# pySTEPS/pysteps

Hardware: NVIDIA H100
Metric: Mpix/s advected (2048^2 frame, 12 leadtimes) (higher is better)
Workload: dtype f64 (trajectories, motion field, IDW); f32 precip in/out; u8/i16/f32 OpenCV-exact LK stages

## Files before the change

### pysteps_b200/csrc/lk_features.cu

```cuda
#include <math_constants.h>

#include "common.cuh"

namespace {

constexpr int TX = 32, TY = 8;

__global__ void __launch_bounds__(256)
masked_max_partial(const float *__restrict__ eig, const uint8_t *__restrict__ valid, size_t N,
                   float *__restrict__ part) {
    __shared__ float sm[8];
    float v = -CUDART_INF_F;
    const size_t stride = (size_t)gridDim.x * blockDim.x;
    for (size_t i = (size_t)blockIdx.x * blockDim.x + threadIdx.x; i < N; i += stride)
        if (!valid || valid[i]) v = fmaxf(v, eig[i]);
#pragma unroll
    for (int o = 16; o > 0; o >>= 1) v = fmaxf(v, __shfl_xor_sync(0xffffffffu, v, o));
    if ((threadIdx.x & 31) == 0) sm[threadIdx.x >> 5] = v;
    __syncthreads();
    if (threadIdx.x < 32) {
        v = threadIdx.x < 8 ? sm[threadIdx.x] : -CUDART_INF_F;
#pragma unroll
        for (int o = 4; o > 0; o >>= 1) v = fmaxf(v, __shfl_xor_sync(0xffffffffu, v, o));
        if (threadIdx.x == 0) part[blockIdx.x] = v;
    }
}

__global__ void __launch_bounds__(256)
masked_max_final(const float *__restrict__ part, int nparts, double quality, unsigned *__restrict__ state) {
    __shared__ float sm[8];
    float v = -CUDART_INF_F;
    for (int i = threadIdx.x; i < nparts; i += blockDim.x) v = fmaxf(v, part[i]);
#pragma unroll
    for (int o = 16; o > 0; o >>= 1) v = fmaxf(v, __shfl_xor_sync(0xffffffffu, v, o));
    if ((threadIdx.x & 31) == 0) sm[threadIdx.x >> 5] = v;
    __syncthreads();
    if (threadIdx.x == 0) {
        for (int i = 1; i < 8; i++) v = fmaxf(v, sm[i]);
        const double mx = (v == -CUDART_INF_F) ? 0.0 : (double)v;
        const float thr = (float)(mx * quality);
        state[0] = __float_as_uint(thr);
        state[1] = 0u;
        state[2] = (v == -CUDART_INF_F) ? 1u : 0u;
    }
}

__device__ __forceinline__ unsigned order_key(float v) {
    const unsigned u = __float_as_uint(v);
    return (u & 0x80000000u) ? ~u : (u | 0x80000000u);
}

__global__ void __launch_bounds__(TX *TY)
candidates_kernel(const float *__restrict__ eig, const uint8_t *__restrict__ valid, int h, int w,
                  unsigned *__restrict__ state, unsigned long long *__restrict__ keys, unsigned cap) {
    const int x = blockIdx.x * TX + threadIdx.x, y = blockIdx.y * TY + threadIdx.y;
    if (x < 1 || y < 1 || x >= w - 1 || y >= h - 1) return;
    const float thr = __uint_as_float(state[0]);
    const size_t i = (size_t)y * w + x;
    const float v = eig[i];
    if (!(v > thr) || v == 0.f) return;
    if (valid && !valid[i]) return;
    bool ismax = true;
#pragma unroll
    for (int dy = -1; dy <= 1; dy++)
#pragma unroll
        for (int dx = -1; dx <= 1; dx++) {
            float u = eig[(size_t)(y + dy) * w + (x + dx)];
            u = (u > thr) ? u : 0.f;
            ismax &= !(u > v);
        }
    if (!ismax) return;
    const unsigned slot = atomicAdd(&state[1], 1u);
    if (slot < cap) keys[slot] = ((unsigned long long)order_key(v) << 32) | (unsigned)i;
}

constexpr int SORT_BLOCK = 1024;
constexpr int SORT_TILE = 2 * SORT_BLOCK;

__device__ __forceinline__ void cmpswap_desc(unsigned long long &a, unsigned long long &b, bool desc) {
    if ((a < b) == desc) {
        const unsigned long long t = a; a = b; b = t;
    }
}

__global__ void __launch_bounds__(SORT_BLOCK)
bitonic_local_kernel(unsigned long long *__restrict__ keys, unsigned n, unsigned k_start, unsigned k_end) {
    __shared__ unsigned long long sm[SORT_TILE];
    const unsigned base = blockIdx.x * SORT_TILE;
    for (unsigned t = threadIdx.x; t < SORT_TILE; t += SORT_BLOCK) sm[t] = (base + t < n) ? keys[base + t] : 0ull;
    __syncthreads();
    for (unsigned k = k_start; k <= k_end; k <<= 1) {
        const unsigned jmax = (k_start == k_end && k_start > SORT_TILE) ? SORT_TILE / 2 : k / 2;
        for (unsigned j = (jmax < k / 2 ? jmax : k / 2); j > 0; j >>= 1) {
            const unsigned t = threadIdx.x;
            const unsigned lo = 2 * t - (t & (j - 1));
            const unsigned hi = lo + j;
            const bool desc = (((base + lo) & k) == 0);
            cmpswap_desc(sm[lo], sm[hi], desc);
            __syncthreads();
        }
    }
    for (unsigned t = threadIdx.x; t < SORT_TILE; t += SORT_BLOCK)
        if (base + t < n) keys[base + t] = sm[t];
}

__global__ void __launch_bounds__(256)
bitonic_global_kernel(unsigned long long *__restrict__ keys, unsigned n, unsigned k, unsigned j) {
    const unsigned t = blockIdx.x * blockDim.x + threadIdx.x;
    if (t >= n / 2) return;
    const unsigned lo = 2 * t - (t & (j - 1));
    const unsigned hi = lo + j;
    const bool desc = ((lo & k) == 0);
    unsigned long long a = keys[lo], b = keys[hi];
    if ((a < b) == desc) { keys[lo] = b; keys[hi] = a; }
}

constexpr int CELL_CAP = 8;

__device__ __forceinline__ bool too_close(float dx, float dy, double md2) {
    return (double)__fadd_rn(__fmul_rn(dx, dx), __fmul_rn(dy, dy)) < md2;
}

struct SelectParams {
    const unsigned long long *keys;
    const unsigned *state;
    unsigned cap;
    int h, w, max_corners;
    double md2;
    bool use_dist;
    int cell, gw, gh;
    int *cell_cnt;
    short2 *cell_pts;
    float *out_xy;
    int *out_count;
};

__global__ void __launch_bounds__(32) select_kernel(const SelectParams p) {
    const int lane = threadIdx.x;
    const unsigned ncand = min(p.state[1], p.cap);
    int accepted = 0;
    const bool limited = p.max_corners > 0;
    for (unsigned basei = 0; basei < ncand; basei += 32) {
        const unsigned ci = basei + lane;
        bool ok = ci < ncand;
        int x = 0, y = 0;
        if (ok) {
            const unsigned addr = (unsigned)(p.keys[ci] & 0xffffffffull);
            y = addr / p.w;
            x = addr - y * p.w;
        }
        const int xc = x / p.cell, yc = y / p.cell;
        if (ok && p.use_dist) {
            const int x1 = max(0, xc - 1), y1 = max(0, yc - 1);
            const int x2 = min(p.gw - 1, xc + 1), y2 = min(p.gh - 1, yc + 1);
            for (int yy = y1; yy <= y2 && ok; yy++)
                for (int xx = x1; xx <= x2 && ok; xx++) {
                    const int c = yy * p.gw + xx;
                    const int cnt = min(p.cell_cnt[c], CELL_CAP);
                    for (int q = 0; q < cnt; q++) {
                        const short2 pt = p.cell_pts[c * CELL_CAP + q];
                        if (too_close((float)(x - pt.x), (float)(y - pt.y), p.md2)) { ok = false; break; }
                    }
                }
        }
        for (int i = 0; i < 32; i++) {
            const bool oki = __shfl_sync(0xffffffffu, ok, i);
            const int xi = __shfl_sync(0xffffffffu, x, i), yi = __shfl_sync(0xffffffffu, y, i);
            if (oki && lane > i && ok && p.use_dist && too_close((float)(x - xi), (float)(y - yi), p.md2))
                ok = false;
        }
        const unsigned bal = __ballot_sync(0xffffffffu, ok);
        const int rank = __popc(bal & ((1u << lane) - 1u));
        const bool take = ok && (!limited || accepted + rank < p.max_corners);
        const int c = yc * p.gw + xc;
        int before = 0;
        for (int i = 0; i < 32; i++) {
            const int ci2 = __shfl_sync(0xffffffffu, c, i);
            const bool ti = __shfl_sync(0xffffffffu, take, i);
            if (ti && i < lane && ci2 == c) before++;
        }
        if (take) {
            const int o = accepted + rank;
            p.out_xy[2 * o] = (float)x;
            p.out_xy[2 * o + 1] = (float)y;
            if (p.use_dist) {
                const int slot = p.cell_cnt[c] + before;
                if (slot < CELL_CAP) p.cell_pts[c * CELL_CAP + slot] = make_short2((short)x, (short)y);
            }
        }
        __syncwarp();
        if (take && p.use_dist) atomicAdd(&p.cell_cnt[c], 1);
        __threadfence_block();
        __syncwarp();
        accepted += __popc(bal);
        if (limited && accepted >= p.max_corners) { accepted = p.max_corners; break; }
    }
    if (lane == 0) *p.out_count = accepted;
}

constexpr int SEL_WARPS = 8;
constexpr unsigned SEL_DONE = 0xffffffffu;

__global__ void __launch_bounds__(32 * SEL_WARPS) select_smem_kernel(const SelectParams p) {
    extern __shared__ unsigned cells[];
    const int lane = threadIdx.x & 31, warp = threadIdx.x >> 5;
    const int ncell = p.gw * p.gh;
    volatile unsigned *ctl = cells + ncell;
    for (int i = threadIdx.x; i < ncell + 2; i += 32 * SEL_WARPS) cells[i] = 0u;
    __syncthreads();
    const unsigned ncand = min(p.state[1], p.cap);
    const unsigned nbatch = (ncand + 31u) / 32u;
    const unsigned md2i = (unsigned)ceil(p.md2);
    const bool limited = p.max_corners > 0;
    for (unsigned b = warp; b < nbatch; b += SEL_WARPS) {
        const unsigned ci = b * 32u + lane;
        bool ok = ci < ncand;
        int x = 0, y = 0;
        if (ok) {
            const unsigned addr = (unsigned)(p.keys[ci] & 0xffffffffull);
            y = addr / p.w;
            x = addr - y * p.w;
        }
        const int xc = x / p.cell, yc = y / p.cell;
        unsigned close = 0u;
#pragma unroll 8
        for (int i = 0; i < 32; i++) {
            const int xi = __shfl_sync(0xffffffffu, x, i), yi = __shfl_sync(0xffffffffu, y, i);
            const int dx = x - xi, dy = y - yi;
            if (i < lane && (unsigned)(dx * dx) + (unsigned)(dy * dy) < md2i) close |= 1u << i;
        }
        int nidx[9];
#pragma unroll
        for (int k = 0; k < 9; k++) {
            const int xx = xc + k % 3 - 1, yy = yc + k / 3 - 1;
            nidx[k] = (ok && xx >= 0 && yy >= 0 && xx < p.gw && yy < p.gh) ? yy * p.gw + xx : -1;
        }
        unsigned tok;
        while ((tok = ctl[0]) != b && tok != SEL_DONE) {}
        if (tok == SEL_DONE) break;
        __syncwarp();
        int accepted = (int)ctl[1];
        unsigned wds[9], any = 0u;
#pragma unroll
        for (int k = 0; k < 9; k++) {
            wds[k] = nidx[k] >= 0 ? cells[nidx[k]] : 0u;
            any |= wds[k];
        }
        if (any) {
#pragma unroll
            for (int k = 0; k < 9; k++) {
                const unsigned wd = wds[k];
                const int cnt = wd & 3u;
                const int ox = (xc + k % 3 - 1) * p.cell, oy = (yc + k / 3 - 1) * p.cell;
                for (int q = 0; q < cnt; q++) {
                    const unsigned f = (wd >> (2 + 10 * q)) & 0x3ffu;
                    if (too_close((float)(x - (ox + (int)(f & 31u))), (float)(y - (oy + (int)(f >> 5))), p.md2))
                        ok = false;
                }
            }
        }
        const unsigned okmask = __ballot_sync(0xffffffffu, ok);
        close &= okmask;
        unsigned acc = __ballot_sync(0xffffffffu, ok && close == 0u);
        unsigned pend = okmask & ~acc;
        while (pend) {
            const int i = __ffs(pend) - 1;
            pend &= pend - 1;
            const bool oki = (__shfl_sync(0xffffffffu, close, i) & acc) == 0u;
            if (oki) acc |= 1u << i;
        }
        ok = (acc >> lane) & 1u;
        const unsigned bal = __ballot_sync(0xffffffffu, ok);
        const int rank = __popc(bal & ((1u << lane) - 1u));
        const bool take = ok && (!limited || accepted + rank < p.max_corners);
        if (take) {
            const int o = accepted + rank;
            p.out_xy[2 * o] = (float)x;
            p.out_xy[2 * o + 1] = (float)y;
        }
        const unsigned tmask = __ballot_sync(0xffffffffu, take);
        const int c = yc * p.gw + xc;
        if (take) {
            const unsigned grp = __match_any_sync(tmask, c);
            if (lane == __ffs(grp) - 1) {
                unsigned wd = cells[c];
                unsigned g = grp;
                while (g) {
                    const int j = __ffs(g) - 1;
                    g &= g - 1;
                    const int xj = __shfl_sync(grp, x, j), yj = __shfl_sync(grp, y, j);
                    const unsigned cnt = wd & 3u;
                    if (cnt < 3u) {
                        const unsigned f = (unsigned)(xj - xc * p.cell) | ((unsigned)(yj - yc * p.cell) << 5);
                        wd = (wd & ~3u) | (f << (2 + 10 * cnt)) | (cnt + 1u);
                    }
                }
                cells[c] = wd;
            } else {
                unsigned g = grp;
                while (g) {
                    const int j = __ffs(g) - 1;
                    g &= g - 1;
                    __shfl_sync(grp, x, j);
                    __shfl_sync(grp, y, j);
                }
            }
        }
        __syncwarp();
        accepted += __popc(bal);
        const bool full = limited && accepted >= p.max_corners;
        if (full) accepted = p.max_corners;
        __threadfence_block();
        if (lane == 0) {
            ctl[1] = (unsigned)accepted;
            __threadfence_block();
            ctl[0] = full ? SEL_DONE : b + 1u;
        }
        if (full) break;
    }
    __syncthreads();
    if (threadIdx.x == 0) *p.out_count = (int)ctl[1];
}

}

extern "C" int b200_good_features(const float *eig, const uint8_t *valid, int m, int n, int max_corners,
                                  double quality_level, double min_distance, float *out_xy,
                                  int *out_count, void *stream) {
    B200_REQUIRE(eig && out_xy && out_count && m >= 1 && n >= 1 && max_corners > 0, "bad arguments");
    B200_REQUIRE((int64_t)m * n < ((int64_t)1 << 31), "image too large");
    cudaStream_t s = (cudaStream_t)stream;
    const size_t N = (size_t)m * n;
    const int nparts = b200::num_sms() * 4;
    b200::Scratch part, state, keys, cellc, cellp;
    B200_CUDA(part.alloc(sizeof(float) * nparts, s));
    B200_CUDA(state.alloc(sizeof(unsigned) * 4, s));
    masked_max_partial<<<nparts, 256, 0, s>>>(eig, valid, N, (float *)part.p);
    B200_LAUNCH_CHECK();
    masked_max_final<<<1, 256, 0, s>>>((const float *)part.p, nparts, quality_level, (unsigned *)state.p);
    B200_LAUNCH_CHECK();
    const unsigned cap = (unsigned)N;
    size_t cap_pow2 = SORT_TILE;
    while (cap_pow2 < (size_t)cap) cap_pow2 <<= 1;
    B200_CUDA(keys.alloc(sizeof(unsigned long long) * cap_pow2, s));
    candidates_kernel<<<dim3(b200::ceil_div(n, TX), b200::ceil_div(m, TY)), dim3(TX, TY), 0, s>>>(
        eig, valid, m, n, (unsigned *)state.p, (unsigned long long *)keys.p, cap);
    B200_LAUNCH_CHECK();
    unsigned hstate[4];
    B200_CUDA(cudaMemcpyAsync(hstate, state.p, sizeof(hstate), cudaMemcpyDeviceToHost, s));
    B200_CUDA(cudaStreamSynchronize(s));
    unsigned ncand = hstate[1] < cap ? hstate[1] : cap;
    if (hstate[2]) ncand = 0;
    if (ncand == 0) {
        B200_CUDA(cudaMemsetAsync(out_count, 0, sizeof(int), s));
        return 0;
    }
    unsigned npow = SORT_TILE;
    while (npow < ncand) npow <<= 1;
    if (npow > ncand)
        B200_CUDA(cudaMemsetAsync((unsigned long long *)keys.p + ncand, 0,
                                  sizeof(unsigned long long) * (npow - ncand), s));
    unsigned long long *K = (unsigned long long *)keys.p;
    bitonic_local_kernel<<<npow / SORT_TILE, SORT_BLOCK, 0, s>>>(K, npow, 2, SORT_TILE);
    B200_LAUNCH_CHECK();
    for (unsigned k = 2 * SORT_TILE; k <= npow; k <<= 1) {
        for (unsigned j = k / 2; j >= SORT_TILE; j >>= 1) {
            bitonic_global_kernel<<<b200::ceil_div((int)(npow / 2), 256), 256, 0, s>>>(K, npow, k, j);
            B200_LAUNCH_CHECK();
        }
        bitonic_local_kernel<<<npow / SORT_TILE, SORT_BLOCK, 0, s>>>(K, npow, k, k);
        B200_LAUNCH_CHECK();
    }
    SelectParams sp;
    sp.keys = K;
    sp.state = (const unsigned *)state.p;
    sp.cap = ncand;
    sp.h = m; sp.w = n;
    sp.max_corners = max_corners;
    sp.md2 = min_distance * min_distance;
    sp.use_dist = min_distance >= 1.0;
    sp.cell = sp.use_dist ? (int)lrint(min_distance) : 1;
    sp.gw = (n + sp.cell - 1) / sp.cell;
    sp.gh = (m + sp.cell - 1) / sp.cell;
    const size_t ncell = (size_t)sp.gw * sp.gh;
    sp.out_xy = out_xy;
    sp.out_count = out_count;
    if (sp.use_dist && sp.cell <= 32 && ncell * sizeof(unsigned) <= 200 * 1024) {
        const size_t smem = (ncell + 2) * sizeof(unsigned);
        B200_CUDA(cudaFuncSetAttribute(select_smem_kernel, cudaFuncAttributeMaxDynamicSharedMemorySize, (int)smem));
        select_smem_kernel<<<1, 32 * SEL_WARPS, smem, s>>>(sp);
        B200_LAUNCH_CHECK();
        return 0;
    }
    B200_CUDA(cellc.alloc(sizeof(int) * ncell, s));
    B200_CUDA(cellp.alloc(sizeof(short2) * ncell * CELL_CAP, s));
    B200_CUDA(cudaMemsetAsync(cellc.p, 0, sizeof(int) * ncell, s));
    sp.cell_cnt = (int *)cellc.p;
    sp.cell_pts = (short2 *)cellp.p;
    sp.out_xy = out_xy;
    sp.out_count = out_count;
    select_kernel<<<1, 32, 0, s>>>(sp);
    B200_LAUNCH_CHECK();
    return 0;
}
```

Before: 19940.

## Replace full bitonic sort of corner candidates with radix top-k chunked selection

The full bitonic sort of every corner candidate is replaced by a radix-histogram top-k pass. It partitions the candidates into those above and those on a 12-bit threshold digit, then sorts only 2048-key chunks in shared memory inside a single fused select kernel. This also removes the device-to-host copy and stream synchronization that used to read the candidate count. The aim is to cut the many global bitonic kernel launches and the host stall in good-features-to-track. In exchange, selection now runs in one block, and every chunk after the first rescans all candidates, which costs more if many chunks are needed.

Result: faster. 20440, median of 6 (+2.5%).

```diff
diff --git a/pysteps_b200/csrc/lk_features.cu b/pysteps_b200/csrc/lk_features.cu
--- a/pysteps_b200/csrc/lk_features.cu
+++ b/pysteps_b200/csrc/lk_features.cu
@@ -5,6 +5,8 @@
 namespace {
 
 constexpr int TX = 32, TY = 8;
+constexpr int RADIX_BITS = 12;
+constexpr unsigned RADIX = 1u << RADIX_BITS;
 
 __global__ void __launch_bounds__(256)
 masked_max_partial(const float *__restrict__ eig, const uint8_t *__restrict__ valid, size_t N,
@@ -31,6 +33,7 @@
     __shared__ float sm[8];
     float v = -CUDART_INF_F;
     for (int i = threadIdx.x; i < nparts; i += blockDim.x) v = fmaxf(v, part[i]);
+    for (int i = 4 + threadIdx.x; i < 8 + (int)RADIX; i += blockDim.x) state[i] = 0u;
 #pragma unroll
     for (int o = 16; o > 0; o >>= 1) v = fmaxf(v, __shfl_xor_sync(0xffffffffu, v, o));
     if ((threadIdx.x & 31) == 0) sm[threadIdx.x >> 5] = v;
@@ -74,45 +77,188 @@
     if (slot < cap) keys[slot] = ((unsigned long long)order_key(v) << 32) | (unsigned)i;
 }
 
-constexpr int SORT_BLOCK = 1024;
-constexpr int SORT_TILE = 2 * SORT_BLOCK;
-
-__device__ __forceinline__ void cmpswap_desc(unsigned long long &a, unsigned long long &b, bool desc) {
-    if ((a < b) == desc) {
-        const unsigned long long t = a; a = b; b = t;
-    }
-}
-
-__global__ void __launch_bounds__(SORT_BLOCK)
-bitonic_local_kernel(unsigned long long *__restrict__ keys, unsigned n, unsigned k_start, unsigned k_end) {
-    __shared__ unsigned long long sm[SORT_TILE];
-    const unsigned base = blockIdx.x * SORT_TILE;
-    for (unsigned t = threadIdx.x; t < SORT_TILE; t += SORT_BLOCK) sm[t] = (base + t < n) ? keys[base + t] : 0ull;
-    __syncthreads();
-    for (unsigned k = k_start; k <= k_end; k <<= 1) {
-        const unsigned jmax = (k_start == k_end && k_start > SORT_TILE) ? SORT_TILE / 2 : k / 2;
-        for (unsigned j = (jmax < k / 2 ? jmax : k / 2); j > 0; j >>= 1) {
-            const unsigned t = threadIdx.x;
-            const unsigned lo = 2 * t - (t & (j - 1));
-            const unsigned hi = lo + j;
-            const bool desc = (((base + lo) & k) == 0);
-            cmpswap_desc(sm[lo], sm[hi], desc);
+constexpr int TOPK_THREADS = 1024;
+constexpr unsigned CHUNK = 2048;
+constexpr int PER_THREAD = RADIX / TOPK_THREADS;
+static_assert(RADIX * sizeof(unsigned) <= CHUNK * sizeof(unsigned long long), "the histogram aliases the chunk");
+static_assert(TOPK_THREADS == 32 * 32, "block_inclusive_scan: one warp scans the warp totals");
+
+constexpr int LOAD_BATCH = 8;
+
+__device__ __forceinline__ void load_keys(const unsigned long long *__restrict__ keys, unsigned ncand, unsigned b,
+                                          unsigned long long (&k)[LOAD_BATCH]) {
+#pragma unroll
+    for (int j = 0; j < LOAD_BATCH; j++) {
+        const unsigned i = b + j * TOPK_THREADS + threadIdx.x;
+        k[j] = i < ncand ? keys[i] : 0ull;
+    }
+}
+
+struct TopkShared {
+    unsigned wsum[32];
+    unsigned digit, above, bucket;
+    unsigned n;
+};
+
+__device__ __forceinline__ unsigned block_inclusive_scan(unsigned v, TopkShared &sh) {
+    const int lane = threadIdx.x & 31, warp = threadIdx.x >> 5;
+#pragma unroll
+    for (int o = 1; o < 32; o <<= 1) {
+        const unsigned t = __shfl_up_sync(0xffffffffu, v, o);
+        if (lane >= o) v += t;
+    }
+    if (lane == 31) sh.wsum[warp] = v;
+    __syncthreads();
+    if (warp == 0) {
+        unsigned w = sh.wsum[lane];
+#pragma unroll
+        for (int o = 1; o < 32; o <<= 1) {
+            const unsigned t = __shfl_up_sync(0xffffffffu, w, o);
+            if (lane >= o) w += t;
+        }
+        sh.wsum[lane] = w;
+    }
+    __syncthreads();
+    return v + (warp ? sh.wsum[warp - 1] : 0u);
+}
+
+__device__ void find_digit(const unsigned *hist, unsigned need, TopkShared &sh) {
+    unsigned c[PER_THREAD], s = 0u;
+#pragma unroll
+    for (int j = 0; j < PER_THREAD; j++) {
+        c[j] = hist[RADIX - 1 - PER_THREAD * threadIdx.x - j];
+        s += c[j];
+    }
+    const unsigned incl = block_inclusive_scan(s, sh);
+    unsigned above = incl - s;
+    if (above < need && incl >= need) {
+#pragma unroll
+        for (int j = 0; j < PER_THREAD; j++) {
+            if (above + c[j] >= need) {
+                sh.digit = RADIX - 1 - PER_THREAD * threadIdx.x - j;
+                sh.above = above;
+                sh.bucket = c[j];
+                break;
+            }
+            above += c[j];
+        }
+    }
+    __syncthreads();
+}
+
+__device__ unsigned long long chunk_bound(const unsigned long long *__restrict__ keys, unsigned nkeys,
+                                          unsigned long long hi, unsigned need, unsigned have, int used,
+                                          unsigned long long prefix, unsigned *hist, TopkShared &sh) {
+    unsigned long long pmask = used ? ~0ull << (64 - used) : 0ull;
+    while (have != need && used < 64) {
+        const int width = min(RADIX_BITS, 64 - used), shift = 64 - used - width;
+        const unsigned dmask = (1u << width) - 1u;
+        for (unsigned i = threadIdx.x; i < RADIX; i += TOPK_THREADS) hist[i] = 0u;
+        __syncthreads();
+        for (unsigned b = 0; b < nkeys; b += LOAD_BATCH * TOPK_THREADS) {
+            unsigned long long k[LOAD_BATCH];
+            load_keys(keys, nkeys, b, k);
+#pragma unroll
+            for (int j = 0; j < LOAD_BATCH; j++)
+                if (k[j] != 0ull && k[j] < hi && (k[j] & pmask) == prefix)
+                    atomicAdd(&hist[(unsigned)(k[j] >> shift) & dmask], 1u);
+        }
+        __syncthreads();
+        find_digit(hist, need, sh);
+        need -= sh.above;
+        have = sh.bucket;
+        prefix |= (unsigned long long)sh.digit << shift;
+        pmask |= (unsigned long long)dmask << shift;
+        used += width;
+        __syncthreads();
+    }
+    return prefix;
+}
+
+__device__ void append_keys(const unsigned long long *__restrict__ keys, unsigned nkeys, unsigned long long lo,
+                            unsigned long long hi, unsigned long long *chunk, TopkShared &sh) {
+    const int lane = threadIdx.x & 31;
+    for (unsigned b = 0; b < nkeys; b += LOAD_BATCH * TOPK_THREADS) {
+        unsigned long long k[LOAD_BATCH];
+        load_keys(keys, nkeys, b, k);
+#pragma unroll
+        for (int j = 0; j < LOAD_BATCH; j++) {
+            const unsigned bal = __ballot_sync(0xffffffffu, k[j] != 0ull && k[j] >= lo && k[j] < hi);
+            unsigned base = 0u;
+            if (lane == 0 && bal) base = atomicAdd(&sh.n, __popc(bal));
+            base = __shfl_sync(0xffffffffu, base, 0);
+            if ((bal >> lane) & 1u) chunk[base + __popc(bal & ((1u << lane) - 1u))] = k[j];
+        }
+    }
+    __syncthreads();
+}
+
+__device__ void sort_chunk(unsigned long long *chunk, unsigned n) {
+    unsigned npow = 2u;
+    while (npow < n) npow <<= 1;
+    for (unsigned i = n + threadIdx.x; i < npow; i += TOPK_THREADS) chunk[i] = 0ull;
+    __syncthreads();
+    for (unsigned k = 2; k <= npow; k <<= 1)
+        for (unsigned j = k >> 1; j > 0; j >>= 1) {
+            for (unsigned t = threadIdx.x; t < npow / 2; t += TOPK_THREADS) {
+                const unsigned a = 2 * t - (t & (j - 1));
+                const bool desc = (a & k) == 0;
+                const unsigned long long x = chunk[a], y = chunk[a + j];
+                if ((x < y) == desc) {
+                    chunk[a] = y;
+                    chunk[a + j] = x;
+                }
+            }
             __syncthreads();
         }
-    }
-    for (unsigned t = threadIdx.x; t < SORT_TILE; t += SORT_BLOCK)
-        if (base + t < n) keys[base + t] = sm[t];
-}
-
-__global__ void __launch_bounds__(256)
-bitonic_global_kernel(unsigned long long *__restrict__ keys, unsigned n, unsigned k, unsigned j) {
-    const unsigned t = blockIdx.x * blockDim.x + threadIdx.x;
-    if (t >= n / 2) return;
-    const unsigned lo = 2 * t - (t & (j - 1));
-    const unsigned hi = lo + j;
-    const bool desc = ((lo & k) == 0);
-    unsigned long long a = keys[lo], b = keys[hi];
-    if ((a < b) == desc) { keys[lo] = b; keys[hi] = a; }
+}
+
+constexpr int TOP_SHIFT = 64 - RADIX_BITS;
+
+__device__ __forceinline__ unsigned candidate_count(const unsigned *state, unsigned cap) {
+    return state[2] ? 0u : min(state[1], cap);
+}
+
+__global__ void __launch_bounds__(TOPK_THREADS)
+key_hist_kernel(const unsigned long long *__restrict__ keys, unsigned *__restrict__ state, unsigned cap) {
+    __shared__ unsigned h[RADIX];
+    const unsigned ncand = candidate_count(state, cap);
+    if (ncand <= CHUNK) return;
+    for (unsigned i = threadIdx.x; i < RADIX; i += TOPK_THREADS) h[i] = 0u;
+    __syncthreads();
+    for (unsigned i = blockIdx.x * TOPK_THREADS + threadIdx.x; i < ncand; i += gridDim.x * TOPK_THREADS)
+        atomicAdd(&h[(unsigned)(keys[i] >> TOP_SHIFT)], 1u);
+    __syncthreads();
+    for (unsigned i = threadIdx.x; i < RADIX; i += TOPK_THREADS)
+        if (h[i]) atomicAdd(&state[8 + i], h[i]);
+}
+
+__global__ void __launch_bounds__(TOPK_THREADS)
+key_partition_kernel(const unsigned long long *__restrict__ keys, unsigned *__restrict__ state, unsigned cap,
+                     unsigned long long *__restrict__ top, unsigned long long *__restrict__ edge) {
+    __shared__ unsigned h[RADIX];
+    __shared__ TopkShared sh;
+    const unsigned ncand = candidate_count(state, cap);
+    if (ncand <= CHUNK) return;
+    for (unsigned i = threadIdx.x; i < RADIX; i += TOPK_THREADS) h[i] = state[8 + i];
+    __syncthreads();
+    find_digit(h, CHUNK, sh);
+    const unsigned d0 = sh.digit;
+    if (blockIdx.x == 0 && threadIdx.x == 0) state[6] = d0;
+    const int lane = threadIdx.x & 31;
+    for (unsigned b = blockIdx.x * TOPK_THREADS; b < ncand; b += gridDim.x * TOPK_THREADS) {
+        const unsigned i = b + threadIdx.x;
+        const unsigned long long k = i < ncand ? keys[i] : 0ull;
+        const unsigned d = (unsigned)(k >> TOP_SHIFT);
+#pragma unroll
+        for (int side = 0; side < 2; side++) {
+            const unsigned bal = __ballot_sync(0xffffffffu, i < ncand && (side ? d == d0 : d > d0));
+            unsigned base = 0u;
+            if (lane == 0 && bal) base = atomicAdd(&state[4 + side], __popc(bal));
+            base = __shfl_sync(0xffffffffu, base, 0);
+            if ((bal >> lane) & 1u) (side ? edge : top)[base + __popc(bal & ((1u << lane) - 1u))] = k;
+        }
+    }
 }
 
 constexpr int CELL_CAP = 8;
@@ -125,6 +271,7 @@
     const unsigned long long *keys;
     const unsigned *state;
     unsigned cap;
+    const unsigned long long *top, *edge;
     int h, w, max_corners;
     double md2;
     bool use_dist;
@@ -135,17 +282,20 @@
     int *out_count;
 };
 
-__global__ void __launch_bounds__(32) select_kernel(const SelectParams p) {
-    const int lane = threadIdx.x;
-    const unsigned ncand = min(p.state[1], p.cap);
-    int accepted = 0;
+constexpr unsigned SEL_DONE = 0xffffffffu;
+
+__device__ void select_chunk_global(const SelectParams &p, const unsigned long long *keys, unsigned ncand,
+                                    volatile unsigned *ctl) {
+    const int lane = threadIdx.x & 31;
+    int accepted = (int)ctl[1];
     const bool limited = p.max_corners > 0;
+    bool full = false;
     for (unsigned basei = 0; basei < ncand; basei += 32) {
         const unsigned ci = basei + lane;
         bool ok = ci < ncand;
         int x = 0, y = 0;
         if (ok) {
-            const unsigned addr = (unsigned)(p.keys[ci] & 0xffffffffull);
+            const unsigned addr = (unsigned)(keys[ci] & 0xffffffffull);
             y = addr / p.w;
             x = addr - y * p.w;
         }
@@ -193,22 +343,19 @@
         __threadfence_block();
         __syncwarp();
         accepted += __popc(bal);
-        if (limited && accepted >= p.max_corners) { accepted = p.max_corners; break; }
-    }
-    if (lane == 0) *p.out_count = accepted;
+        if (limited && accepted >= p.max_corners) { accepted = p.max_corners; full = true; break; }
+    }
+    if (lane == 0) {
+        ctl[1] = (unsigned)accepted;
+        if (full) ctl[0] = SEL_DONE;
+    }
 }
 
 constexpr int SEL_WARPS = 8;
-constexpr unsigned SEL_DONE = 0xffffffffu;
-
-__global__ void __launch_bounds__(32 * SEL_WARPS) select_smem_kernel(const SelectParams p) {
-    extern __shared__ unsigned cells[];
+
+__device__ void select_chunk_smem(const SelectParams &p, const unsigned long long *keys, unsigned ncand,
+                                  unsigned *cells, volatile unsigned *ctl) {
     const int lane = threadIdx.x & 31, warp = threadIdx.x >> 5;
-    const int ncell = p.gw * p.gh;
-    volatile unsigned *ctl = cells + ncell;
-    for (int i = threadIdx.x; i < ncell + 2; i += 32 * SEL_WARPS) cells[i] = 0u;
-    __syncthreads();
-    const unsigned ncand = min(p.state[1], p.cap);
     const unsigned nbatch = (ncand + 31u) / 32u;
     const unsigned md2i = (unsigned)ceil(p.md2);
     const bool limited = p.max_corners > 0;
@@ -217,7 +364,7 @@
         bool ok = ci < ncand;
         int x = 0, y = 0;
         if (ok) {
-            const unsigned addr = (unsigned)(p.keys[ci] & 0xffffffffull);
+            const unsigned addr = (unsigned)(keys[ci] & 0xffffffffull);
             y = addr / p.w;
             x = addr - y * p.w;
         }
@@ -318,6 +465,52 @@
         }
         if (full) break;
     }
+}
+
+template <bool SMEM_GRID>
+__global__ void __launch_bounds__(TOPK_THREADS) topk_select_kernel(const SelectParams p) {
+    extern __shared__ unsigned long long chunk[];
+    unsigned *cells = (unsigned *)(chunk + CHUNK);
+    __shared__ TopkShared sh;
+    __shared__ unsigned ctl_words[2];
+    volatile unsigned *ctl = ctl_words;
+    if (SMEM_GRID)
+        for (int i = threadIdx.x; i < p.gw * p.gh; i += TOPK_THREADS) cells[i] = 0u;
+    if (threadIdx.x == 0) ctl[0] = ctl[1] = 0u;
+    __syncthreads();
+    const unsigned ncand = candidate_count(p.state, p.cap);
+    unsigned long long hi = ~0ull;
+    for (unsigned rem = ncand; rem > 0;) {
+        if (threadIdx.x == 0) sh.n = 0u;
+        __syncthreads();
+        unsigned long long lo = 0ull;
+        if (rem <= CHUNK) {
+            append_keys(p.keys, ncand, 0ull, hi, chunk, sh);
+        } else if (rem == ncand) {
+            const unsigned above = p.state[4], nedge = p.state[5];
+            lo = chunk_bound(p.edge, nedge, hi, CHUNK - above, nedge, RADIX_BITS,
+                             (unsigned long long)p.state[6] << TOP_SHIFT, (unsigned *)chunk, sh);
+            append_keys(p.top, above, 0ull, hi, chunk, sh);
+            append_keys(p.edge, nedge, lo, hi, chunk, sh);
+        } else {
+            lo = chunk_bound(p.keys, ncand, hi, CHUNK, rem, 0, 0ull, (unsigned *)chunk, sh);
+            append_keys(p.keys, ncand, lo, hi, chunk, sh);
+        }
+        const unsigned n = sh.n;
+        sort_chunk(chunk, n);
+        const int warp = threadIdx.x >> 5;
+        if (SMEM_GRID) {
+            if (warp < SEL_WARPS) select_chunk_smem(p, chunk, n, cells, ctl);
+        } else if (warp == 0) {
+            select_chunk_global(p, chunk, n, ctl);
+        }
+        __syncthreads();
+        if (ctl[0] == SEL_DONE) break;
+        __syncthreads();
+        if (threadIdx.x == 0) ctl[0] = 0u;
+        hi = lo;
+        rem -= n;
+    }
     __syncthreads();
     if (threadIdx.x == 0) *p.out_count = (int)ctl[1];
 }
@@ -332,49 +525,32 @@
     cudaStream_t s = (cudaStream_t)stream;
     const size_t N = (size_t)m * n;
     const int nparts = b200::num_sms() * 4;
-    b200::Scratch part, state, keys, cellc, cellp;
+    b200::Scratch part, state, keys, top, edge, cellc, cellp;
     B200_CUDA(part.alloc(sizeof(float) * nparts, s));
-    B200_CUDA(state.alloc(sizeof(unsigned) * 4, s));
+    B200_CUDA(state.alloc(sizeof(unsigned) * (8 + RADIX), s));
     masked_max_partial<<<nparts, 256, 0, s>>>(eig, valid, N, (float *)part.p);
     B200_LAUNCH_CHECK();
     masked_max_final<<<1, 256, 0, s>>>((const float *)part.p, nparts, quality_level, (unsigned *)state.p);
     B200_LAUNCH_CHECK();
     const unsigned cap = (unsigned)N;
-    size_t cap_pow2 = SORT_TILE;
-    while (cap_pow2 < (size_t)cap) cap_pow2 <<= 1;
-    B200_CUDA(keys.alloc(sizeof(unsigned long long) * cap_pow2, s));
+    B200_CUDA(keys.alloc(sizeof(unsigned long long) * cap, s));
+    B200_CUDA(top.alloc(sizeof(unsigned long long) * CHUNK, s));
+    B200_CUDA(edge.alloc(sizeof(unsigned long long) * cap, s));
     candidates_kernel<<<dim3(b200::ceil_div(n, TX), b200::ceil_div(m, TY)), dim3(TX, TY), 0, s>>>(
         eig, valid, m, n, (unsigned *)state.p, (unsigned long long *)keys.p, cap);
     B200_LAUNCH_CHECK();
-    unsigned hstate[4];
-    B200_CUDA(cudaMemcpyAsync(hstate, state.p, sizeof(hstate), cudaMemcpyDeviceToHost, s));
-    B200_CUDA(cudaStreamSynchronize(s));
-    unsigned ncand = hstate[1] < cap ? hstate[1] : cap;
-    if (hstate[2]) ncand = 0;
-    if (ncand == 0) {
-        B200_CUDA(cudaMemsetAsync(out_count, 0, sizeof(int), s));
-        return 0;
-    }
-    unsigned npow = SORT_TILE;
-    while (npow < ncand) npow <<= 1;
-    if (npow > ncand)
-        B200_CUDA(cudaMemsetAsync((unsigned long long *)keys.p + ncand, 0,
-                                  sizeof(unsigned long long) * (npow - ncand), s));
-    unsigned long long *K = (unsigned long long *)keys.p;
-    bitonic_local_kernel<<<npow / SORT_TILE, SORT_BLOCK, 0, s>>>(K, npow, 2, SORT_TILE);
+    const int kgrid = 32;
+    key_hist_kernel<<<kgrid, TOPK_THREADS, 0, s>>>((const unsigned long long *)keys.p, (unsigned *)state.p, cap);
     B200_LAUNCH_CHECK();
-    for (unsigned k = 2 * SORT_TILE; k <= npow; k <<= 1) {
-        for (unsigned j = k / 2; j >= SORT_TILE; j >>= 1) {
-            bitonic_global_kernel<<<b200::ceil_div((int)(npow / 2), 256), 256, 0, s>>>(K, npow, k, j);
-            B200_LAUNCH_CHECK();
-        }
-        bitonic_local_kernel<<<npow / SORT_TILE, SORT_BLOCK, 0, s>>>(K, npow, k, k);
-        B200_LAUNCH_CHECK();
-    }
+    key_partition_kernel<<<kgrid, TOPK_THREADS, 0, s>>>((const unsigned long long *)keys.p, (unsigned *)state.p, cap,
+                                                        (unsigned long long *)top.p, (unsigned long long *)edge.p);
+    B200_LAUNCH_CHECK();
     SelectParams sp;
-    sp.keys = K;
+    sp.keys = (const unsigned long long *)keys.p;
     sp.state = (const unsigned *)state.p;
-    sp.cap = ncand;
+    sp.cap = cap;
+    sp.top = (const unsigned long long *)top.p;
+    sp.edge = (const unsigned long long *)edge.p;
     sp.h = m; sp.w = n;
     sp.max_corners = max_corners;
     sp.md2 = min_distance * min_distance;
@@ -385,21 +561,25 @@
     const size_t ncell = (size_t)sp.gw * sp.gh;
     sp.out_xy = out_xy;
     sp.out_count = out_count;
+    sp.cell_cnt = nullptr;
+    sp.cell_pts = nullptr;
+    const size_t chunk_bytes = sizeof(unsigned long long) * CHUNK;
     if (sp.use_dist && sp.cell <= 32 && ncell * sizeof(unsigned) <= 200 * 1024) {
-        const size_t smem = (ncell + 2) * sizeof(unsigned);
-        B200_CUDA(cudaFuncSetAttribute(select_smem_kernel, cudaFuncAttributeMaxDynamicSharedMemorySize, (int)smem));
-        select_smem_kernel<<<1, 32 * SEL_WARPS, smem, s>>>(sp);
+        const size_t smem = chunk_bytes + ncell * sizeof(unsigned);
+        B200_CUDA(cudaFuncSetAttribute(topk_select_kernel<true>, cudaFuncAttributeMaxDynamicSharedMemorySize,
+                                       (int)smem));
+        topk_select_kernel<true><<<1, TOPK_THREADS, smem, s>>>(sp);
         B200_LAUNCH_CHECK();
         return 0;
     }
-    B200_CUDA(cellc.alloc(sizeof(int) * ncell, s));
-    B200_CUDA(cellp.alloc(sizeof(short2) * ncell * CELL_CAP, s));
-    B200_CUDA(cudaMemsetAsync(cellc.p, 0, sizeof(int) * ncell, s));
-    sp.cell_cnt = (int *)cellc.p;
-    sp.cell_pts = (short2 *)cellp.p;
-    sp.out_xy = out_xy;
-    sp.out_count = out_count;
-    select_kernel<<<1, 32, 0, s>>>(sp);
+    if (sp.use_dist) {
+        B200_CUDA(cellc.alloc(sizeof(int) * ncell, s));
+        B200_CUDA(cellp.alloc(sizeof(short2) * ncell * CELL_CAP, s));
+        B200_CUDA(cudaMemsetAsync(cellc.p, 0, sizeof(int) * ncell, s));
+        sp.cell_cnt = (int *)cellc.p;
+        sp.cell_pts = (short2 *)cellp.p;
+    }
+    topk_select_kernel<false><<<1, TOPK_THREADS, chunk_bytes, s>>>(sp);
     B200_LAUNCH_CHECK();
     return 0;
 }
```

## Make good-features pipeline device-driven with fused max and cluster/cooperative bitonic sort

Applied to the files above, without the earlier changes.

Merges the two-kernel masked max into one kernel using a last-block atomic reduction. Removes the host readback and stream synchronize of the candidate count, so sort sizes are decided on device. The many per-stage sort launches become one thread-block-cluster kernel (distributed shared memory, 8 CTAs) for small candidate sets, or one cooperative grid-sync kernel for large ones. Shared-memory passes now do radix-8 strides with a swizzle. The cost is extra grid/cluster syncs and a cooperative launch, and the sort kernels must size npow from device state each call.

Result: no change. 20410 before, 20380 after, median of 6 (-0.1%).

```diff
diff --git a/pysteps_b200/csrc/lk_features.cu b/pysteps_b200/csrc/lk_features.cu
--- a/pysteps_b200/csrc/lk_features.cu
+++ b/pysteps_b200/csrc/lk_features.cu
@@ -1,48 +1,56 @@
+#include <cooperative_groups.h>
 #include <math_constants.h>
 
 #include "common.cuh"
 
+namespace cg = cooperative_groups;
+
 namespace {
 
 constexpr int TX = 32, TY = 8;
 
+__device__ __forceinline__ float block_max(float v, float *sm) {
+#pragma unroll
+    for (int o = 16; o > 0; o >>= 1) v = fmaxf(v, __shfl_xor_sync(0xffffffffu, v, o));
+    __syncthreads();
+    if ((threadIdx.x & 31) == 0) sm[threadIdx.x >> 5] = v;
+    __syncthreads();
+    v = sm[0];
+    for (int i = 1; i < 8; i++) v = fmaxf(v, sm[i]);
+    return v;
+}
+
 __global__ void __launch_bounds__(256)
-masked_max_partial(const float *__restrict__ eig, const uint8_t *__restrict__ valid, size_t N,
-                   float *__restrict__ part) {
+masked_max_kernel(const float *__restrict__ eig, const uint8_t *__restrict__ valid, size_t N,
+                  float *__restrict__ part, double quality, unsigned *__restrict__ state) {
     __shared__ float sm[8];
+    __shared__ int s_last;
     float v = -CUDART_INF_F;
     const size_t stride = (size_t)gridDim.x * blockDim.x;
     for (size_t i = (size_t)blockIdx.x * blockDim.x + threadIdx.x; i < N; i += stride)
         if (!valid || valid[i]) v = fmaxf(v, eig[i]);
-#pragma unroll
-    for (int o = 16; o > 0; o >>= 1) v = fmaxf(v, __shfl_xor_sync(0xffffffffu, v, o));
-    if ((threadIdx.x & 31) == 0) sm[threadIdx.x >> 5] = v;
-    __syncthreads();
-    if (threadIdx.x < 32) {
-        v = threadIdx.x < 8 ? sm[threadIdx.x] : -CUDART_INF_F;
-#pragma unroll
-        for (int o = 4; o > 0; o >>= 1) v = fmaxf(v, __shfl_xor_sync(0xffffffffu, v, o));
-        if (threadIdx.x == 0) part[blockIdx.x] = v;
-    }
-}
-
-__global__ void __launch_bounds__(256)
-masked_max_final(const float *__restrict__ part, int nparts, double quality, unsigned *__restrict__ state) {
-    __shared__ float sm[8];
-    float v = -CUDART_INF_F;
-    for (int i = threadIdx.x; i < nparts; i += blockDim.x) v = fmaxf(v, part[i]);
-#pragma unroll
-    for (int o = 16; o > 0; o >>= 1) v = fmaxf(v, __shfl_xor_sync(0xffffffffu, v, o));
-    if ((threadIdx.x & 31) == 0) sm[threadIdx.x >> 5] = v;
-    __syncthreads();
+    v = block_max(v, sm);
     if (threadIdx.x == 0) {
-        for (int i = 1; i < 8; i++) v = fmaxf(v, sm[i]);
+        part[blockIdx.x] = v;
+        __threadfence();
+        s_last = atomicAdd(&state[3], 1u) == gridDim.x - 1;
+    }
+    __syncthreads();
+    if (!s_last) return;
+    __threadfence();
+    v = -CUDART_INF_F;
+    for (int i = threadIdx.x; i < gridDim.x; i += blockDim.x) v = fmaxf(v, __ldcg(&part[i]));
+    v = block_max(v, sm);
+    if (threadIdx.x == 0) {
         const double mx = (v == -CUDART_INF_F) ? 0.0 : (double)v;
         const float thr = (float)(mx * quality);
         state[0] = __float_as_uint(thr);
-        state[1] = 0u;
         state[2] = (v == -CUDART_INF_F) ? 1u : 0u;
     }
+}
+
+__device__ __forceinline__ unsigned candidate_count(const unsigned *state, unsigned cap) {
+    return state[2] ? 0u : min(state[1], cap);
 }
 
 __device__ __forceinline__ unsigned order_key(float v) {
@@ -75,7 +83,9 @@
 }
 
 constexpr int SORT_BLOCK = 1024;
-constexpr int SORT_TILE = 2 * SORT_BLOCK;
+constexpr unsigned SORT_TILE = 8192;
+constexpr int CL_CTAS = 8;
+constexpr unsigned CL_KEYS = CL_CTAS * SORT_TILE;
 
 __device__ __forceinline__ void cmpswap_desc(unsigned long long &a, unsigned long long &b, bool desc) {
     if ((a < b) == desc) {
@@ -83,36 +93,117 @@
     }
 }
 
+__device__ __forceinline__ unsigned sw(unsigned i) { return i ^ ((i >> 3) & 7u); }
+
+template <int L>
+__device__ __forceinline__ void strides_pass(unsigned long long *sm, unsigned n, unsigned base, unsigned k,
+                                             unsigned j) {
+    constexpr int G = 1 << L;
+    const unsigned jl = j >> (L - 1);
+    for (unsigned t = threadIdx.x; t < n / G; t += SORT_BLOCK) {
+        const unsigned p0 = ((t & ~(jl - 1)) << L) | (t & (jl - 1));
+        const bool desc = (((base + p0) & k) == 0);
+        unsigned long long v[G];
+#pragma unroll
+        for (int m = 0; m < G; m++) v[m] = sm[sw(p0 + m * jl)];
+#pragma unroll
+        for (int st = G / 2; st > 0; st >>= 1)
+#pragma unroll
+            for (int m = 0; m < G; m++)
+                if (!(m & st)) cmpswap_desc(v[m], v[m + st], desc);
+#pragma unroll
+        for (int m = 0; m < G; m++) sm[sw(p0 + m * jl)] = v[m];
+    }
+    __syncthreads();
+}
+
+__device__ __forceinline__ void smem_strides(unsigned long long *sm, unsigned n, unsigned base, unsigned k,
+                                             unsigned jtop) {
+    for (unsigned j = min(k / 2, jtop); j > 0;) {
+        if (j >= 4) {
+            strides_pass<3>(sm, n, base, k, j);
+            j >>= 3;
+        } else if (j == 2) {
+            strides_pass<2>(sm, n, base, k, j);
+            j = 0;
+        } else {
+            strides_pass<1>(sm, n, base, k, j);
+            j = 0;
+        }
+    }
+}
+
+__device__ void bitonic_tile(unsigned long long *keys, unsigned long long *sm, unsigned base, unsigned lim,
+                             unsigned k_start, unsigned k_end) {
+    __syncthreads();
+    for (unsigned t = threadIdx.x; t < SORT_TILE; t += SORT_BLOCK)
+        sm[sw(t)] = (base + t < lim) ? __ldcg(&keys[base + t]) : 0ull;
+    __syncthreads();
+    for (unsigned k = k_start; k <= k_end; k <<= 1) smem_strides(sm, SORT_TILE, base, k, SORT_TILE / 2);
+    for (unsigned t = threadIdx.x; t < SORT_TILE; t += SORT_BLOCK) __stcg(&keys[base + t], sm[sw(t)]);
+}
+
+__global__ void __cluster_dims__(CL_CTAS, 1, 1) __launch_bounds__(SORT_BLOCK)
+sort_cluster_kernel(unsigned long long *keys, const unsigned *__restrict__ state, unsigned cap) {
+    extern __shared__ unsigned long long cl_sm[];
+    const unsigned ncand = candidate_count(state, cap);
+    if (ncand <= 1 || ncand > CL_KEYS) return;
+    cg::cluster_group cluster = cg::this_cluster();
+    unsigned npow = 2;
+    while (npow < ncand) npow <<= 1;
+    const unsigned seg = min(npow, SORT_TILE);
+    const unsigned r = cluster.block_rank(), base = r * seg;
+    const bool active = base < npow;
+    if (active) {
+        for (unsigned t = threadIdx.x; t < seg; t += SORT_BLOCK) cl_sm[sw(t)] = (base + t < ncand) ? keys[base + t] : 0ull;
+        __syncthreads();
+        for (unsigned k = 2; k <= seg; k <<= 1) smem_strides(cl_sm, seg, base, k, seg / 2);
+    }
+    for (unsigned k = 2 * seg; k <= npow; k <<= 1) {
+        for (unsigned j = k / 2; j >= seg; j >>= 1) {
+            cluster.sync();
+            if (active) {
+                const bool is_lo = (r & (j / seg)) == 0;
+                unsigned long long *other = cluster.map_shared_rank(cl_sm, r ^ (j / seg));
+                unsigned long long *lo_sm = is_lo ? cl_sm : other, *hi_sm = is_lo ? other : cl_sm;
+                const unsigned lo_base = is_lo ? base : base - j;
+                for (unsigned e = threadIdx.x + (is_lo ? 0u : seg / 2); e < (is_lo ? seg / 2 : seg); e += SORT_BLOCK)
+                    cmpswap_desc(lo_sm[sw(e)], hi_sm[sw(e)], ((lo_base + e) & k) == 0);
+            }
+            cluster.sync();
+        }
+        if (active) smem_strides(cl_sm, seg, base, k, seg / 2);
+    }
+    if (active)
+        for (unsigned t = threadIdx.x; t < seg; t += SORT_BLOCK) keys[base + t] = cl_sm[sw(t)];
+}
+
 __global__ void __launch_bounds__(SORT_BLOCK)
-bitonic_local_kernel(unsigned long long *__restrict__ keys, unsigned n, unsigned k_start, unsigned k_end) {
-    __shared__ unsigned long long sm[SORT_TILE];
-    const unsigned base = blockIdx.x * SORT_TILE;
-    for (unsigned t = threadIdx.x; t < SORT_TILE; t += SORT_BLOCK) sm[t] = (base + t < n) ? keys[base + t] : 0ull;
-    __syncthreads();
-    for (unsigned k = k_start; k <= k_end; k <<= 1) {
-        const unsigned jmax = (k_start == k_end && k_start > SORT_TILE) ? SORT_TILE / 2 : k / 2;
-        for (unsigned j = (jmax < k / 2 ? jmax : k / 2); j > 0; j >>= 1) {
-            const unsigned t = threadIdx.x;
-            const unsigned lo = 2 * t - (t & (j - 1));
-            const unsigned hi = lo + j;
-            const bool desc = (((base + lo) & k) == 0);
-            cmpswap_desc(sm[lo], sm[hi], desc);
-            __syncthreads();
-        }
-    }
-    for (unsigned t = threadIdx.x; t < SORT_TILE; t += SORT_BLOCK)
-        if (base + t < n) keys[base + t] = sm[t];
-}
-
-__global__ void __launch_bounds__(256)
-bitonic_global_kernel(unsigned long long *__restrict__ keys, unsigned n, unsigned k, unsigned j) {
-    const unsigned t = blockIdx.x * blockDim.x + threadIdx.x;
-    if (t >= n / 2) return;
-    const unsigned lo = 2 * t - (t & (j - 1));
-    const unsigned hi = lo + j;
-    const bool desc = ((lo & k) == 0);
-    unsigned long long a = keys[lo], b = keys[hi];
-    if ((a < b) == desc) { keys[lo] = b; keys[hi] = a; }
+sort_keys_kernel(unsigned long long *keys, const unsigned *__restrict__ state, unsigned cap) {
+    extern __shared__ unsigned long long sort_sm[];
+    const unsigned ncand = candidate_count(state, cap);
+    if (ncand <= CL_KEYS) return;
+    unsigned npow = SORT_TILE;
+    while (npow < ncand) npow <<= 1;
+    const unsigned ntiles = npow / SORT_TILE;
+    cg::grid_group grid = cg::this_grid();
+    for (unsigned tl = blockIdx.x; tl < ntiles; tl += gridDim.x)
+        bitonic_tile(keys, sort_sm, tl * SORT_TILE, ncand, 2, SORT_TILE);
+    const unsigned stride = gridDim.x * SORT_BLOCK;
+    for (unsigned k = 2 * SORT_TILE; k <= npow; k <<= 1) {
+        for (unsigned j = k / 2; j >= SORT_TILE; j >>= 1) {
+            grid.sync();
+            for (unsigned t = blockIdx.x * SORT_BLOCK + threadIdx.x; t < npow / 2; t += stride) {
+                const unsigned lo = 2 * t - (t & (j - 1));
+                const bool desc = ((lo & k) == 0);
+                const unsigned long long a = __ldcg(&keys[lo]), b = __ldcg(&keys[lo + j]);
+                if ((a < b) == desc) { __stcg(&keys[lo], b); __stcg(&keys[lo + j], a); }
+            }
+        }
+        grid.sync();
+        for (unsigned tl = blockIdx.x; tl < ntiles; tl += gridDim.x)
+            bitonic_tile(keys, sort_sm, tl * SORT_TILE, npow, k, k);
+    }
 }
 
 constexpr int CELL_CAP = 8;
@@ -137,7 +228,7 @@
 
 __global__ void __launch_bounds__(32) select_kernel(const SelectParams p) {
     const int lane = threadIdx.x;
-    const unsigned ncand = min(p.state[1], p.cap);
+    const unsigned ncand = candidate_count(p.state, p.cap);
     int accepted = 0;
     const bool limited = p.max_corners > 0;
     for (unsigned basei = 0; basei < ncand; basei += 32) {
@@ -208,7 +299,7 @@
     volatile unsigned *ctl = cells + ncell;
     for (int i = threadIdx.x; i < ncell + 2; i += 32 * SEL_WARPS) cells[i] = 0u;
     __syncthreads();
-    const unsigned ncand = min(p.state[1], p.cap);
+    const unsigned ncand = candidate_count(p.state, p.cap);
     const unsigned nbatch = (ncand + 31u) / 32u;
     const unsigned md2i = (unsigned)ceil(p.md2);
     const bool limited = p.max_corners > 0;
@@ -335,9 +426,8 @@
     b200::Scratch part, state, keys, cellc, cellp;
     B200_CUDA(part.alloc(sizeof(float) * nparts, s));
     B200_CUDA(state.alloc(sizeof(unsigned) * 4, s));
-    masked_max_partial<<<nparts, 256, 0, s>>>(eig, valid, N, (float *)part.p);
-    B200_LAUNCH_CHECK();
-    masked_max_final<<<1, 256, 0, s>>>((const float *)part.p, nparts, quality_level, (unsigned *)state.p);
+    B200_CUDA(cudaMemsetAsync(state.p, 0, sizeof(unsigned) * 4, s));
+    masked_max_kernel<<<nparts, 256, 0, s>>>(eig, valid, N, (float *)part.p, quality_level, (unsigned *)state.p);
     B200_LAUNCH_CHECK();
     const unsigned cap = (unsigned)N;
     size_t cap_pow2 = SORT_TILE;
@@ -346,35 +436,30 @@
     candidates_kernel<<<dim3(b200::ceil_div(n, TX), b200::ceil_div(m, TY)), dim3(TX, TY), 0, s>>>(
         eig, valid, m, n, (unsigned *)state.p, (unsigned long long *)keys.p, cap);
     B200_LAUNCH_CHECK();
-    unsigned hstate[4];
-    B200_CUDA(cudaMemcpyAsync(hstate, state.p, sizeof(hstate), cudaMemcpyDeviceToHost, s));
-    B200_CUDA(cudaStreamSynchronize(s));
-    unsigned ncand = hstate[1] < cap ? hstate[1] : cap;
-    if (hstate[2]) ncand = 0;
-    if (ncand == 0) {
-        B200_CUDA(cudaMemsetAsync(out_count, 0, sizeof(int), s));
-        return 0;
-    }
-    unsigned npow = SORT_TILE;
-    while (npow < ncand) npow <<= 1;
-    if (npow > ncand)
-        B200_CUDA(cudaMemsetAsync((unsigned long long *)keys.p + ncand, 0,
-                                  sizeof(unsigned long long) * (npow - ncand), s));
     unsigned long long *K = (unsigned long long *)keys.p;
-    bitonic_local_kernel<<<npow / SORT_TILE, SORT_BLOCK, 0, s>>>(K, npow, 2, SORT_TILE);
-    B200_LAUNCH_CHECK();
-    for (unsigned k = 2 * SORT_TILE; k <= npow; k <<= 1) {
-        for (unsigned j = k / 2; j >= SORT_TILE; j >>= 1) {
-            bitonic_global_kernel<<<b200::ceil_div((int)(npow / 2), 256), 256, 0, s>>>(K, npow, k, j);
+    {
+        const int smem = SORT_TILE * sizeof(unsigned long long);
+        B200_CUDA(cudaFuncSetAttribute(sort_cluster_kernel, cudaFuncAttributeMaxDynamicSharedMemorySize, smem));
+        sort_cluster_kernel<<<CL_CTAS, SORT_BLOCK, smem, s>>>(K, (const unsigned *)state.p, cap);
+        B200_LAUNCH_CHECK();
+        if (cap > CL_KEYS) {
+            B200_CUDA(cudaFuncSetAttribute(sort_keys_kernel, cudaFuncAttributeMaxDynamicSharedMemorySize, smem));
+            int per_sm = 0;
+            B200_CUDA(cudaOccupancyMaxActiveBlocksPerMultiprocessor(&per_sm, sort_keys_kernel, SORT_BLOCK, smem));
+            B200_REQUIRE(per_sm >= 1, "sort kernel does not fit on an SM");
+            const unsigned grid = (unsigned)std::min<size_t>((size_t)b200::num_sms(), cap_pow2 / SORT_TILE);
+            const unsigned *st = (const unsigned *)state.p;
+            unsigned cap_arg = cap;
+            void *args[] = {&K, &st, &cap_arg};
+            B200_CUDA(cudaLaunchCooperativeKernel((const void *)sort_keys_kernel, dim3(grid), dim3(SORT_BLOCK), args,
+                                                  (size_t)smem, s));
             B200_LAUNCH_CHECK();
         }
-        bitonic_local_kernel<<<npow / SORT_TILE, SORT_BLOCK, 0, s>>>(K, npow, k, k);
-        B200_LAUNCH_CHECK();
     }
     SelectParams sp;
     sp.keys = K;
     sp.state = (const unsigned *)state.p;
-    sp.cap = ncand;
+    sp.cap = cap;
     sp.h = m; sp.w = n;
     sp.max_corners = max_corners;
     sp.md2 = min_distance * min_distance;
```
